# AIRI-Institute/HairFastGAN

Measured on AMD Instinct MI355X. Metric: stylegan2_generator_fwd_1024_images_per_sec, higher is better.
Workload: dtype f32 tensors + f32 accumulate; conv products as 3 fp16 MFMAs on (hi,lo)-split operands (fp32-class); 1 GPU; StyleGAN2 1024^2 generator forward (range 0->8), random W+, fresh noise per layer, HIP modulated-conv + upfirdn2d kernels (BASELINE.json configs[1]); batch_per_gpu=8, global_batch=8, parallelism=replica x1, weights=synthetic closed-form (oracle/synth.py), conv_precision=f16x3

## Files before the change

hairfastgan_amd/_lib.py:

```python
import ctypes
import os

_HERE = os.path.dirname(os.path.abspath(__file__))
LIB_PATH = os.environ.get("HAIRFAST_HIP_LIB") or os.path.join(_HERE, "csrc", "libhairfast_hip.so")

_f = ctypes.c_void_p
_i = ctypes.c_int
_ll = ctypes.c_longlong
_fl = ctypes.c_float
_st = ctypes.c_void_p

SIGNATURES = {
    "hf_upfirdn2d_f32": [_f, _f, _f, _i, _i, _i, _i, _i, _i, _i, _i, _i, _i, _i, _i, _i, _st],
    "hf_fused_bias_act_f32": [_f, _f, _f, _ll, _i, _i, _fl, _fl, _st],
    "hf_noise_bias_act_f32": [_f, _f, _f, _f, _f, _i, _i, _i, _ll, _fl, _fl, _st],
    "hf_modconv_prepare_f32": [_f, _f, _f, _i, _i, _i, _st],
    "hf_modulation_f32": [_f, _f, _ll, _f, _f, _i, _i, _i, _st],
    "hf_style_batch_f32": [_f, _f, _ll, _ll, _f, _i, _i, _i, _i, _i, _st],
    "hf_demod_f32": [_f, _f, _f, _i, _i, _i, _st],
    "hf_style_normalize_f32": [_f, _f, _i, _i, _i, _st],
    "hf_modconv3x3_f32": [_f, _f, _f, _f, _f, _f, _f, _ll, _f, _i, _i, _i, _i, _i, _fl, _fl, _f, _ll, _st],
    "hf_conv_split_weights_f16": [_f, _f, _f, _i, _i, _st],
    "hf_conv_split_weights_f16_taps": [_f, _f, _f, _i, _i, _i, _st],
    "hf_modconv3x3_small_f16_f32": [_f, _f, _f, _f, _i, _f, _f, _f, _f, _ll, _f, _i, _i, _i, _i, _i, _fl, _fl, _i, _i, _f, _ll, _st],
    "hf_modconv3x3_small_up_blur_f16_f32": [_f, _f, _f, _f, _f, _f, _i, _f, _f, _f, _f, _f, _ll, _f, _f, _i, _i, _i, _i, _i, _fl, _fl, _f, _ll, _st],
    "hf_conv1x1_f16_f32": [_f, _f, _f, _f, _f, _f, _i, _f, _f, _f, _f, _i, _f, _fl, _f, _i, _i, _i, _i, _i, _i, _i, _ll, _f, _ll, _st],
    "hf_modconv3x3_f16_f32": [_f, _f, _f, _f, _i, _f, _f, _f, _f, _ll, _f, _i, _i, _i, _i, _i, _fl, _fl, _st],
    "hf_modconv3x3_f16_rgb_f32": [_f, _f, _f, _f, _i, _f, _f, _f, _f, _ll, _f, _i, _i, _i, _i, _i, _fl, _fl, _f, _f, _f, _st],
    "hf_modconv3x3_f16_pre_image_f32": [_f, _f, _f, _f, _f, _i, _f, _f, _f, _ll, _f, _i, _i, _i, _i, _i, _fl, _fl, _f, _f, _f, _f, _f, _st],
    "hf_modconv3x3_f16_pre_f32": [_f, _f, _f, _f, _f, _i, _f, _f, _f, _ll, _f, _i, _i, _i, _i, _i, _fl, _fl, _f, _f, _f, _f, _f, _f, _st],
    "hf_modconv3x3_up_f16_pre_f32": [_f, _f, _f, _f, _f, _i, _f, _i, _i, _i, _i, _i, _i, _st],
    "hf_modconv3x3_up_f16_f32": [_f, _f, _f, _f, _i, _f, _f, _i, _i, _i, _i, _i, _i, _st],
    "hf_modconv3x3_up_blur_f16_f32": [_f, _f, _f, _f, _f, _f, _f, _f, _f, _f, ctypes.POINTER(ctypes.c_float),
                                      ctypes.POINTER(ctypes.c_float), _f, _f, _ll, _f, _f, _i, _i, _i, _i, _i, _fl, _fl, _st],
    "hf_modconv3x3_up_f32": [_f, _f, _f, _f, _f, _i, _i, _i, _i, _i, _i, _f, _ll, _st],
    "hf_modconv_up_pitch": [_i],
    "hf_blur_noise_bias_act_f32": [_f, _f, _f, _f, _f, _ll, _f, _i, _i, _i, _i, _i, _fl, _fl, _st],
    "hf_blur_noise_bias_act_split_f16": [_f, _f, _f, _f, _f, _f, _ll, _f, _f, _i, _i, _i, _i, _i, _fl, _fl, _st],
    "hf_torgb_f32": [_f, _f, _f, _f, _f, _f, _f, _i, _i, _i, _i, _st],
    "hf_conv_prepare_f32": [_f, _f, _i, _i, _i, _fl, _st],
    "hf_bn_fold_f32": [_f, _f, _f, _f, _f, _f, _f, _fl, _i, _st],
    "hf_conv2d_f32": [_f, _f, _f, _f, _f, _f, _f, _i, _f, _fl, _f, _i, _i, _i, _i, _i, _i, _i, _i, _ll, _f, _ll, _st],
    "hf_conv2d_f16_f32": [_f, _f, _f, _f, _f, _f, _i, _f, _f, _f, _f, _i, _f, _fl, _f, _i, _i, _i, _i, _i, _i, _i, _ll, _f, _ll, _st],
    "hf_split_activation_f16": [_f, _f, _f, _f, _f, _ll, _i, _i, _i, _st],
    "hf_split_activation_mod_f16": [_f, _f, _f, _f, _ll, _i, _i, _i, _st],
    "hf_plane_mean_f32": [_f, _f, _i, _i, _st],
    "hf_se_gate_f32": [_f, _f, _f, _f, _i, _i, _i, _st],
    "hf_scale_shortcut_add_f32": [_f, _f, _f, _f, _i, _i, _i, _i, _i, _i, _i, _st],
    "hf_upsample_bilinear_add_f32": [_f, _f, _f, _i, _i, _i, _i, _i, _st],
    "hf_adaptive_avgpool_f32": [_f, _f, _i, _i, _i, _i, _i, _i, _i, _i, _st],
    "hf_downscale2x_f32": [_f, _f, _i, _i, _i, _st],
    "hf_linear_f32": [_f, _f, _ll, _f, _f, _i, _i, _i, _fl, _st],
    "hf_equal_linear_f32": [_f, _f, _ll, _f, _f, _i, _i, _i, _fl, _i, _fl, _fl, _st],
    "hf_pixel_norm_f32": [_f, _f, _i, _i, _st],
    "hf_bicubic_down_f32": [_f, _f, _f, _ll, _i, _i, _i, _st],
    "hf_dilate_erode_f32": [_f, _f, _f, _ll, _i, _i, _i, _st],
    "hf_quantize_u8_f32": [_f, _f, _ll, _st],
    "hf_poisson_setup_u8": [_f, _f, _f, _f, _f, _i, _i, _i, _i, _st],
    "hf_poisson_jacobi_f32": [_f, _f, _f, _f, _i, _i, _i, _i, _i, _i, _st],
    "hf_poisson_finish_u8": [_f, _f, _f, _f, _i, _i, _i, _i, _st],
    "hf_resize_lanczos_u8": [_f, _f, _f, _i, _i, _i, _i, _i, _f, _f, _i, _f, _f, _i, _st],
    "hf_quad_bilinear_u8": [_f, _f, ctypes.POINTER(ctypes.c_double), _i, _i, _i, _i, _i, _st],
    "hf_quad_lanczos4_u8": [_f, _f, ctypes.POINTER(ctypes.c_double), _i, _i, _i, _i, _f, _f, _i, _st],
    "hf_quad_lanczos4_ratio": [],
    "hf_align_pad_blur_f32": [_f, _f, _f, _f, _i, _f, _f, _i, _i, _i, _i, _i, _i, _i, _st],
    "hf_align_pad_finish_u8": [_f, _f, _f, _f, _f, _f, _i, _i, _i, _st],
    "hf_u8_to_unit_f32": [_f, _f, _ll, _st],
    "hf_image_to_bytes_f32": [_f, _f, _i, _i, _i, _fl, _fl, _i, _i, _st],
    "hf_labels_to_rgb_i64": [_f, _f, _ll, _f, _i, _i, _st],
    "hf_maxpool3x3s2_f32": [_f, _f, _ll, _i, _i, _st],
    "hf_gate_f32": [_f, _f, _f, _f, _f, _fl, _ll, _i, _st],
    "hf_upsample_nearest_f32": [_f, _f, _ll, _i, _i, _i, _i, _st],
    "hf_parsing_mask_i64": [_f, _f, _f, _i, _i, _i, _i, _i, _i, _i, _i, _st],
    "hf_layernorm_f32": [_f, _f, _f, _f, _i, _i, _fl, _i, _fl, _st],
    "hf_layernorm_grouped_f32": [_f, _f, _f, _f, _i, _i, _i, _fl, _i, _fl, _st],
    "hf_modulate_f32": [_f, _f, _f, _f, _ll, _i, _fl, _st],
    "hf_sample_layernorm_f32": [_f, _f, _f, _f, _i, _i, _i, _ll, _fl, _fl, _f, _ll, _st],
    "hf_pixel_norm_dim1_f32": [_f, _f, _i, _i, _i, _st],
    "hf_axpby_bcast_f32": [_f, _f, _fl, _f, _fl, _ll, _ll, _st],
    "hf_add_bcast_f32": [_f, _f, _f, _ll, _ll, _st],
    "hf_label_conv3x3_f32": [_f, _f, _f, _f, _i, _i, _i, _i, _i, _i, _i, _i, _f, _st],
    "hf_ace_modulate_f32": [_f, _f, _f, _f, _f, _f, _f, _f, _f, _i, _i, _i, _i, _fl, _i, _st],
    "hf_conv2d_f16_split_f32": [_f, _f, _f, _f, _f, _f, _f, _f, _f, _f, _i, _f, _f, _f, _f, _i, _f, _fl, _f, _i, _i, _i, _i, _i, _i, _st],
    "hf_stem7x7s2_f16_f32": [_f, _f, _f, _f, _f, _f, _f, _fl, _i, _i, _i, _i, _i, _st],
    "hf_ace_modulate_table_f32": [_f, _f, _f, _f, _f, _f, _f, _f, _f, _f, _f, _i, _i, _i, _i, _i, _i, _i, _fl, _i, _i, _st],
    "hf_region_mean_f32": [_f, _f, _f, _i, _i, _i, _i, _i, _ll, _ll, _i, _i, _st],
    "hf_tanh_f32": [_f, _f, _ll, _st],
    "hf_channel_layernorm_f32": [_f, _f, _f, _f, _i, _ll, _fl, _st],
    "hf_mha_small_f32": [_f, _f, _i, _i, _i, _i, _st],
    "hf_quick_gelu_f32": [_f, _f, _ll, _st],
    "hf_debug_set_dispatch": [_i, _i],
    "hf_debug_last_path": [],
    "hf_debug_set_persistent_blocks": [_i],
    "hf_debug_set_tuning": [_i],
    "hf_set_batch_invariant": [_i],
    "hf_set_splitk_counters": [_f, _i],
# ... 49 lines not shown
```

hairfastgan_amd/_marshal.py:

```python
import functools
import os

import torch
import torch.nn.functional as F

from ._lib import check
from ._runtime import CANON_BATCH, plan_batch

SQRT2 = 2 ** 0.5

PROFILE = None


KERNEL_NAMES = {
    211: "conv_mfma_pipe<2,2,2,4>", 212: "conv_mfma_pipe<2,2,1,4>", 213: "conv_mfma_pipe<1,2,1,4>",
    214: "conv_mfma_pipe<2,2,2,2>", 215: "conv_mfma_pipe<1,1,2,2>", 216: "conv_mfma_pipe<1,4,1,4>",
    231: "conv_mfma_dma<2,2,2,4>", 232: "conv_mfma_dma<2,2,1,4>", 233: "conv_mfma_dma<1,2,1,4>", 234: "conv_mfma_dma<2,2,2,2>",
    244: "conv_mfma_pipe<2,2,2,2,stride2>", 245: "conv_mfma_pipe<1,1,2,2,stride2>",
    221: "conv_mfma_pipe<1,2,2,2,up>", 222: "conv_mfma_pipe<1,2,1,4,up>", 223: "conv_mfma_pipe<1,1,2,2,up>",
    224: "conv_mfma_pipe<1,2,2,4,up>", 225: "conv_mfma_pipe<1,1,1,4,up>", 300: "conv_mfma<1,1,2,2> split-K",
    581: "conv_mfma_h<1,2,2,4,up,pre>", 583: "conv_mfma_h<1,2,1,8,up,pre>",
    571: "conv_mfma_h<1,2,2,4,pre>", 572: "conv_mfma_h<2,2,1,8,pre>", 575: "conv_mfma_h<1,2,1,8,tw128,pre>",
    579: "conv_rows_h<32->32,strip64,pre>",
    551: "conv_mfma_h<1,2,2,4>", 552: "conv_mfma_h<2,2,1,8>", 553: "conv_mfma_h<1,2,1,8>", 555: "conv_mfma_h<1,2,1,8,tw128>",
# ... 326 lines not shown
    return out, raw, split


def modconv3x3_f16_pre(lib, st, act, wt_hi, wt_lo, nterms, d, noise, noise_w, bias, alpha=0.2, scale=SQRT2, rgb=None,
                       want_out=True, split_for=None):
    out, raw, split = _modconv3x3_f16_pre(lib, st, act, wt_hi, wt_lo, nterms, d, noise, noise_w, bias, alpha, scale, rgb, want_out,
                                          split_for)
    res = (out,) + (() if rgb is None else (raw,)) + (() if split_for is None else (split,))
    return res[0] if len(res) == 1 else res


def split_weights_small(lib, st, wt):
    taps, cin, cout = wt.shape
    w1 = _c(wt).permute(1, 0, 2).reshape(1, cin, taps * cout).contiguous()
    return conv_split_weights_f16(lib, st, w1)


def modconv3x3_small_supported(cin, cout, h, w, batch, upsample=False):
    if cin % 32 or cout % 64 or h * w > 1024:
        return False
    n = plan_batch(batch) * h * w
    if upsample:
        return h * w <= 64 or (h * w <= 256 and n <= 1024)
    return 256 < n <= 2048 or (n == 256 and h * w <= 64) or (h * w == 64 and CANON_BATCH * 64 <= n <= 2048)


def conv3x3_small_supported(cin, cout, h, w, batch):
    return cin % 32 == 0 and cout % 64 == 0 and h * w <= 256 and plan_batch(batch) * h * w <= 4096 and cin * cout >= 512 * 512


def modconv3x3_small(lib, st, x, w9, nterms, s, d, noise, noise_w, bias, cout, alpha=0.2, scale=SQRT2, upsample=False):
    x = _c(x)
    b, cin, h, w = x.shape
    hi, lo = w9
    n = lib.hf_modconv3x3_small_workspace_floats(b, cin, cout, h, w)
    ws = x.new_empty((max(n, 1),))
    if upsample:
        pitch = lib.hf_modconv_up_pitch(w)
        out = x.new_empty((b, cout, 2 * h + 1, pitch))
        noise = bias = noise_w = None
        nbs = 0
    else:
        pitch = 0
        out = x.new_empty((b, cout, h, w))
        noise, nbs = _noise_args(noise, b, h * w)
    code = _launch_profiled(
        lib, 2.0 * cin * cout * 9 * h * w * b,
        lambda: lib.hf_modconv3x3_small_f16_f32(_p(out), _p(x), _p(hi), _p(lo), nterms, _p(_c(s)), _p(_c(d)), _p(noise),
                                                _p(_c(noise_w)), nbs, _p(_c(bias)), b, cin, cout, h, w, alpha, scale,
                                                1 if upsample else 0, pitch, _p(ws), n, st),
        label="gemm_h tap-GEMM (small planes)")
    check(lib, code, "hf_modconv3x3_small_f16_f32")
    return out


SMALL_UP_FUSED = os.environ.get("HAIRFAST_SMALL_UP_FUSED", "1") != "0"


def small_up_blur_supported(h, w):
    return (8 * (2 * h + 3) * (2 * w + 3) + 72 * h * w) * 4 <= 150 * 1024


def modconv3x3_small_up_blur(lib, st, x, w9, nterms, s, d, blur_kernel, noise, noise_w, bias, cout, alpha=0.2, scale=SQRT2,
                             split_for=None):
    x = _c(x)
    b, cin, h, w = x.shape
    hi, lo = w9
    n = lib.hf_modconv3x3_small_workspace_floats(b, cin, cout, h, w)
    ws = x.new_empty((max(n, 1),))
    noise, nbs = _noise_args(noise, b, 4 * h * w)
    out = split = s_next = None
    if split_for is not None:
        s_next = _c(split_for[1])
        split = SplitActivation.empty(b, cout, 2 * h, 2 * w, x.device, want_lo=split_for[2] if len(split_for) > 2 else True,
                                      key=split_for[0])
    else:
        out = x.new_empty((b, cout, 2 * h, 2 * w))
    code = _launch_profiled(
        lib, 2.0 * cin * cout * 9 * h * w * b,
        lambda: lib.hf_modconv3x3_small_up_blur_f16_f32(_p(out), *_hl(split), _p(x), _p(hi), _p(lo), nterms, _p(_c(s)), _p(_c(d)),
                                                        _p(_c(blur_kernel)), _p(noise), _p(_c(noise_w)), nbs, _p(_c(bias)),
                                                        _p(s_next), b, cin, cout, h, w, alpha, scale, _p(ws), n, st),
        label="gemm_h tap-GEMM (small planes)")
    check(lib, code, "hf_modconv3x3_small_up_blur_f16_f32")
    return out if split_for is None else split


def modconv3x3_up_f16_supported(cin, cout, h, w, batch=None):
    if batch is not None and plan_batch(batch) * h * w < 512:
        return False
    return cin % 16 == 0 and cout % 32 == 0 and h * w >= (256 if cout % 64 == 0 else 512) and min(h, w) >= 2


def modconv3x3_up(lib, st, x, wt, s, d, blur_kernel, noise, noise_w, bias, alpha=0.2, scale=SQRT2, f16=None,
                  split_for=None, small=None):
    pre = isinstance(x, SplitActivation)
    if not pre:
        x = _c(x)
    b, cin, h, w = x.shape
    cout = wt.shape[2]
    pitch = lib.hf_modconv_up_pitch(w)
    if pre or small is None:
        tmp = torch.empty((b, cout, 2 * h + 1, pitch), dtype=torch.float32, device=(x.hi if pre else x).device)
    if pre:
        hi, lo, nterms = f16
        code = _launch_profiled(
# ... 811 lines not shown
```

hairfastgan_amd/csrc/api.hip:

```cpp
#include "hf_common.h"

extern "C" const char *hf_strerror(int code) {
  switch (code) {
    case HF_OK: return "ok";
    case HF_E_INVALID: return "invalid argument";
    case HF_E_LAUNCH: return "kernel launch failed";
    case HF_E_WORKSPACE: return "workspace too small";
    default: return "unknown error";
  }
}

extern "C" int hf_abi_version(void) { return 13; }

__global__ void hf_profile_marker_kernel() {}

extern "C" int hf_profile_marker(int id, void *stream) {
  if (id < 0 || id > 1023) return HF_E_INVALID;
  hipLaunchKernelGGL(hf_profile_marker_kernel, dim3(id + 1), dim3(64), 0, static_cast<hipStream_t>(stream));
  return hipGetLastError() == hipSuccess ? HF_OK : HF_E_LAUNCH;
}

extern "C" unsigned long long hf_f16_overflow_count_convh(int reset);
extern "C" unsigned long long hf_f16_overflow_count_blur(int reset);
extern "C" unsigned long long hf_f16_overflow_count_enc(int reset);
extern "C" unsigned long long hf_f16_overflow_count_gemm(int reset);
extern "C" unsigned long long hf_f16_overflow_count_stem(int reset);

extern "C" long long hf_f16_overflow_count(int reset) {
  return (long long)(hf_f16_overflow_count_convh(reset) + hf_f16_overflow_count_blur(reset) + hf_f16_overflow_count_enc(reset) +
                     hf_f16_overflow_count_gemm(reset) + hf_f16_overflow_count_stem(reset));
}
```

hairfastgan_amd/stylegan2/model.py:

```python
import math
import os
import random

import torch
from torch import nn
from torch.nn import functional as F

from .. import _marshal as M
from .._runtime import conv_nterms, conv_precision, lib, reference_rng_walk, require_gpu, run_guarded, stream
from .op import FusedLeakyReLU, fused_leaky_relu, upfirdn2d


FUSE_BLUR_MIN_H = int(os.environ.get("HAIRFAST_FUSE_BLUR_MIN_H", "128"))


class PixelNorm(nn.Module):
    def forward(self, input):
        require_gpu(input)
        return M.pixel_norm(lib(), stream(), input)


def make_kernel(k):
    k = torch.tensor(k, dtype=torch.float32)
    if k.ndim == 1:
# ... 72 lines not shown
        self.upsample = upsample
        self.downsample = downsample
        if upsample:
            factor = 2
            p = (len(blur_kernel) - factor) - (kernel_size - 1)
            self.blur = Blur(blur_kernel, pad=((p + 1) // 2 + factor - 1, p // 2 + 1), upsample_factor=factor)
        self.scale = 1 / math.sqrt(in_channel * kernel_size ** 2)
        self.padding = kernel_size // 2
        self.weight = nn.Parameter(torch.randn(1, out_channel, in_channel, kernel_size, kernel_size))
        self.modulation = EqualLinear(style_dim, in_channel, bias_init=1)
        self.demodulate = demodulate
        self._prep = None
        self._prep_f16 = None
        self._coeffs = None
        self.register_load_state_dict_post_hook(lambda m, _ik: m.invalidate())

    def invalidate(self):
        self._prep = self._prep_f16 = self._coeffs = None

    def __repr__(self):
        return (f"{self.__class__.__name__}({self.in_channel}, {self.out_channel}, {self.kernel_size}, "
                f"upsample={self.upsample}, downsample={self.downsample})")

    def prepared(self):
        w = self.weight
        key = (w.data_ptr(), None if w.is_inference() else w._version, w.device)
        if self._prep is None or self._prep[0] != key:
            require_gpu(w)
            wt, wsq = M.prepare_weights(lib(), stream(), w.detach())
            self._prep = (key, wt, wsq)
        return self._prep[1], self._prep[2]

    def prepared_f16(self):
        wt, _ = self.prepared()
        key = self._prep[0]
        if self._prep_f16 is None or self._prep_f16[0] != key:
            hi, lo = M.split_weights_f16(lib(), stream(), wt)
            self._prep_f16 = (key, hi, lo)
        return self._prep_f16[1], self._prep_f16[2]

    def prepared_small(self):
        wt, _ = self.prepared()
        key = self._prep[0]
        cached = self.__dict__.get("_prep_small")
        if cached is None or cached[0] != key:
            cached = self.__dict__["_prep_small"] = (key, M.split_weights_small(lib(), stream(), wt))
        return cached[1]

    def route_same_res(self, shape, plain=True):
        b, cin, h, w = shape
        cout = self.out_channel
        if conv_precision() == "f32":
            return "f32", False
        if plain and M.modconv3x3_small_supported(cin, cout, h, w, b):
            return "small", False
        if M.modconv3x3_f16_supported(cin, cout, h, w, batch=b):
            return "f16", not self.upsample and self.kernel_size == 3 and M.torgb_fusable(cin, cout, h, w)
        return "f32", False

    def route_up(self, shape, is_split=False, tail=True):
        b, cin, h, w = shape
        cout = self.out_channel
        if conv_precision() == "f32":
            return "f32"
        if h >= FUSE_BLUR_MIN_H and tail and M.modconv3x3_up_fused_supported(cin, cout, h, w) and self.blur_factors() is not None:
            return "fused"
        if not is_split and M.modconv3x3_small_supported(cin, cout, h, w, b, upsample=True):
            return "small"
        return "f16" if M.modconv3x3_up_f16_supported(cin, cout, h, w, batch=b) else "f32"

    def conv_same_res(self, input, wt, s, d, noise, noise_w, bias, alpha=0.2, scale=math.sqrt(2), rgb=None):
        kernel, _ = self.route_same_res(input.shape, plain=rgb is None)
        if kernel == "small":
            return M.modconv3x3_small(lib(), stream(), input, self.prepared_small(), conv_nterms(), s, d, noise, noise_w, bias,
                                      self.out_channel, alpha, scale)
        if kernel == "f16":
            hi, lo = self.prepared_f16()
            return M.modconv3x3_f16(lib(), stream(), input, hi, lo, conv_nterms(), s, d, noise, noise_w, bias, alpha, scale, rgb=rgb)
        assert rgb is None
        return M.modconv3x3(lib(), stream(), input, wt, s, d, noise, noise_w, bias, alpha, scale)

    def fuses_torgb(self, input):
        return self.route_same_res(input.shape, plain=False)[1]

    def blur_factors(self):
        k = self.blur.kernel
        key = (k.data_ptr(), k._version if not k.is_inference() else None)
        cached = self.__dict__.get("_blur_fac")
        if cached is None or cached[0] != key:
            if torch.cuda.is_current_stream_capturing():
                return None if cached is None else cached[1]
            cached = self.__dict__["_blur_fac"] = (key, M.blur_factors(k))
        return cached[1]

    def conv_up(self, input, wt, s, d, noise, noise_w, bias, alpha=0.2, scale=math.sqrt(2), split_for=None):
        route = self.route_up(input.shape, isinstance(input, M.SplitActivation),
                              tail=noise is not None and bias is not None and 0.0 <= alpha <= 1.0)
        if route == "fused":
            hi, lo = self.prepared_f16()
            return M.modconv3x3_up_fused(lib(), stream(), input, hi, lo, s, d, self.blur_factors(), noise, noise_w, bias, alpha, scale,
                                         split_for=None if split_for is None else split_for[1], nterms=conv_nterms())
        f16 = small = None
        if route == "small":
            small = (self.prepared_small(), conv_nterms())
        elif route == "f16":
            f16 = (*self.prepared_f16(), conv_nterms())
        return M.modconv3x3_up(lib(), stream(), input, wt, s, d, self.blur.kernel, noise, noise_w, bias, alpha, scale,
                               f16=f16, split_for=split_for, small=small)

    def style_coefficients(self, style):
        pre = self._coeffs
        if pre is not None and pre[0] == (style.data_ptr(), tuple(style.shape), tuple(style.stride())):
            return pre[1]
        wt, wsq = self.prepared()
        s = M.modulation(lib(), stream(), style, self.modulation.weight.detach(), self.modulation.bias.detach())
        d = None
        if self.demodulate:
            d = M.demod(lib(), stream(), s, wsq)
            M.style_normalize(lib(), stream(), s, d)
        return wt, s, d

    def forward(self, input, style):
        require_gpu(input, style)
        wt, s, d = self.style_coefficients(style)
        if self.kernel_size == 1:
            return M.torgb(lib(), stream(), input, wt, s, None, None, None)
        if self.upsample:
            if tuple(self.blur.pad) != (1, 1) or tuple(self.blur.kernel.shape) != (4, 4):
                raise NotImplementedError("fused upsampling path expects the [1,3,3,1] blur with pad (1,1)")
            return self.conv_up(input, wt, s, d, None, None, None)
        return self.conv_same_res(input, wt, s, d, None, None, None)


# ... 28 lines not shown
        self.noise = NoiseInjection()
        self.activate = FusedLeakyReLU(out_channel)

    def forward(self, input, style, noise=None):
        return self._run(input, style, noise, None)

    def forward_rgb(self, input, style, noise, rgb):
        return self._run(input, style, noise, rgb)

    def _run(self, input, style, noise, rgb):
        require_gpu(input, style, noise)
        conv = self.conv
        wt, s, d = conv.style_coefficients(style)
        b, _, h, w = input.shape
        oh, ow = (2 * h, 2 * w) if conv.upsample else (h, w)
        if noise is None:
            noise = input.new_empty(b, 1, oh, ow).normal_()
        act = self.activate
        if conv.upsample:
            assert rgb is None
            return conv.conv_up(input, wt, s, d, noise, self.noise.weight.detach(), act.bias.detach(),
                                act.negative_slope, act.scale)
        if rgb is None:
            return conv.conv_same_res(input, wt, s, d, noise, self.noise.weight.detach(), act.bias.detach(),
                                      act.negative_slope, act.scale)
        rgb_wt, rgb_s = rgb
        return conv.conv_same_res(input, wt, s, d, noise, self.noise.weight.detach(), act.bias.detach(),
                                  act.negative_slope, act.scale, rgb=(rgb_wt, rgb_s))

    def forward_split(self, input, style, noise, s_next, coeffs=None):
        pre = isinstance(input, M.SplitActivation)
        require_gpu(None if pre else input, style, noise)
        conv = self.conv
        assert conv.upsample
        wt, s, d = conv.style_coefficients(style) if coeffs is None else coeffs
        b, _, h, w = input.shape
        if noise is None:
            noise = style.new_empty(b, 1, 2 * h, 2 * w).normal_()
        act = self.activate
        return conv.conv_up(input, wt, s, d, noise, self.noise.weight.detach(), act.bias.detach(),
                            act.negative_slope, act.scale, split_for=(None, s_next, conv_precision() == "f16x3"))

    def forward_image(self, split, coeffs, noise, rgb, to_rgb, skip):
        conv, act = self.conv, self.activate
        _, s, d = coeffs
        b, _, h, w = split.shape
        if noise is None:
            noise = split.hi.new_empty(b, 1, h, w, dtype=torch.float32).normal_()
        require_gpu(noise, skip)
        hi, lo = conv.prepared_f16()
        return M.modconv3x3_f16_pre_image(lib(), stream(), split, hi, lo, conv_nterms(), d, noise, self.noise.weight.detach(),
                                          act.bias.detach(), rgb, to_rgb.bias.detach(), skip, to_rgb._skip_kernel(skip),
                                          act.negative_slope, act.scale)

    def forward_from_split(self, split, coeffs, noise=None, rgb=None, want_out=True, split_for=None):
        conv = self.conv
        assert not conv.upsample
        _, s, d = coeffs
        b, _, h, w = split.shape
        if noise is None:
            noise = split.hi.new_empty(b, 1, h, w, dtype=torch.float32).normal_()
        require_gpu(noise)
        act = self.activate
        hi, lo = conv.prepared_f16()
        return M._modconv3x3_f16_pre(lib(), stream(), split, hi, lo, conv_nterms(), d, noise, self.noise.weight.detach(),
                                     act.bias.detach(), act.negative_slope, act.scale, rgb=rgb, want_out=want_out,
                                     split_for=split_for)


def _observed(*modules):
    for m in modules:
        for sub in m.modules():
            if sub._forward_hooks or sub._forward_pre_hooks:
                return True
    return False


class ToRGB(nn.Module):
    def __init__(self, in_channel, style_dim, upsample=True, blur_kernel=[1, 3, 3, 1]):
        super().__init__()
        if upsample:
            self.upsample = Upsample(blur_kernel)
        self.conv = ModulatedConv2d(in_channel, 3, 1, style_dim, demodulate=False)
        self.bias = nn.Parameter(torch.zeros(1, 3, 1, 1))

    def _skip_kernel(self, skip):
        if skip is None:
            return None
        kern = self.upsample.kernel
        if tuple(kern.shape) != (4, 4) or self.upsample.factor != 2 or tuple(self.upsample.pad) != (2, 1):
            raise NotImplementedError("fused skip path expects the [1,3,3,1] x2 upsampler")
        return kern

    def forward(self, input, style, skip=None):
        require_gpu(input, style, skip)
        wt, s, _ = self.conv.style_coefficients(style)
        return M.torgb(lib(), stream(), input, wt, s, self.bias.detach(), skip, self._skip_kernel(skip))

    def coefficients(self, style):
        wt, s, _ = self.conv.style_coefficients(style)
        return wt, s

    def finish(self, raw, skip=None):
        require_gpu(raw, skip)
        slabs = raw.shape[1] // 3
        eye = getattr(self, "_eye", None)
# ... 130 lines not shown
        res = M.style_batch(lib(), stream(), lat, table, layout, total, mci, mco)
        for conv, row, (sv, dv) in zip(convs, rows, res):
            view = latent[:, row]
            conv._coeffs = ((view.data_ptr(), tuple(view.shape), tuple(view.stride())), (conv.prepared()[0], sv, dv))
        return convs

    def _fast_block(self, block, src, mid_shape, fuses, latent, noise, skip, up_coeffs, end_layer):
        conv_up, conv_same, to_rgb = self.convs[2 * block - 2], self.convs[2 * block - 1], self.to_rgbs[block - 1]
        i = 2 * block - 1
        coeffs = conv_same.conv.style_coefficients(latent[:, i + 1])
        split = conv_up.forward_split(src, latent[:, i], noise[2 * block - 1], coeffs[1],
                                      coeffs=up_coeffs if isinstance(src, M.SplitActivation) else None)
        rgb = to_rgb.coefficients(latent[:, i + 2]) if fuses else None
        is_last = block == self.log_size - 2
        s_up = None
        if not is_last and block + 1 <= end_layer:
            nup, nsame = self.convs[2 * block], self.convs[2 * block + 1]
            up_shape = (mid_shape[0], conv_same.conv.out_channel) + mid_shape[2:]
            next_mid = (mid_shape[0], nup.conv.out_channel, 2 * mid_shape[2], 2 * mid_shape[3])
            if (nup.conv.route_up(up_shape, is_split=True) != "f32" and nsame.conv.route_same_res(next_mid, plain=False)[0] == "f16"
                    and not _observed(nup, nsame)):
                up_coeffs = nup.conv.style_coefficients(latent[:, i + 2])
                s_up = up_coeffs[1]
        fused_rgb = rgb is not None and not _observed(to_rgb)
        want_out = not fused_rgb or (not is_last and s_up is None)
        if (fused_rgb and not want_out and s_up is None and skip is not None and M.image_fusable(mid_shape[1], conv_same.conv.out_channel, *mid_shape[2:])
                and conv_same.activate.bias is not None):
            image = conv_same.forward_image(split, coeffs, noise[2 * block], rgb, to_rgb, skip)
            if image is not None:
                return None, image, None, up_coeffs
        out, raw, split_in = conv_same.forward_from_split(split, coeffs, noise[2 * block], rgb=rgb if fused_rgb else None,
                                                          want_out=want_out, split_for=s_up)
        skip = to_rgb.finish(raw, skip) if raw is not None else to_rgb(out, latent[:, i + 2], skip)
        return out, skip, split_in, up_coeffs

    def _run_layers(self, latent, noise, layer_in, skip, start_layer, end_layer, return_latents):
        out = self.input(latent)
        if start_layer == 0:
            out = self.conv1(out, latent[:, 0], noise=noise[0])
            skip = self.to_rgb1(out, latent[:, 1])
        if end_layer == 0:
            return out, skip
        split_in = up_coeffs = None
        for block in range(1, self.log_size - 1):
            if block < start_layer:
                continue
            if block != start_layer and block > end_layer:
                return out, skip
            conv_up, conv_same, to_rgb = self.convs[2 * block - 2], self.convs[2 * block - 1], self.to_rgbs[block - 1]
            i = 2 * block - 1
            src = layer_in if block == start_layer else (split_in if split_in is not None else out)
            mid_shape = (src.shape[0], conv_up.conv.out_channel, 2 * src.shape[2], 2 * src.shape[3])
            kernel, fuses = conv_same.conv.route_same_res(mid_shape, plain=False)
            if kernel == "f16" and not _observed(conv_up, conv_same):
                out, skip, split_in, up_coeffs = self._fast_block(block, src, mid_shape, fuses, latent, noise, skip, up_coeffs, end_layer)
            else:
                assert not isinstance(src, M.SplitActivation)
                split_in = None
                out = conv_up(src, latent[:, i], noise=noise[2 * block - 1])
                if fuses and not _observed(conv_same, to_rgb):
                    out, raw = conv_same.forward_rgb(out, latent[:, i + 1], noise[2 * block], to_rgb.coefficients(latent[:, i + 2]))
                    skip = to_rgb.finish(raw, skip)
                else:
                    out = conv_same(out, latent[:, i + 1], noise=noise[2 * block])
                    skip = to_rgb(out, latent[:, i + 2], skip)
        image = skip
        return (image, latent) if return_latents else (image, None)
```

include/hairfast_hip.h:

```cpp
#ifndef HAIRFAST_HIP_H
#define HAIRFAST_HIP_H

#ifdef __cplusplus
extern "C" {
#endif

#define HF_OK 0
#define HF_E_INVALID (-1)
#define HF_E_LAUNCH (-2)
#define HF_E_WORKSPACE (-3)

#define HF_ACT_RESIDUAL_FIRST 16

const char *hf_strerror(int code);
int hf_abi_version(void);

int hf_upfirdn2d_f32(float *out, const float *in, const float *kernel, int major, int in_h, int in_w,
                     int kh, int kw, int up_x, int up_y, int down_x, int down_y, int pad_x0, int pad_x1,
                     int pad_y0, int pad_y1, void *stream);

int hf_fused_bias_act_f32(float *out, const float *x, const float *bias, long long n, int n_bias,
                          int step_b, float alpha, float scale, void *stream);

int hf_noise_bias_act_f32(float *out, const float *x, const float *noise, const float *noise_w,
// ... 79 lines not shown
                                     const float *noise, const float *noise_w, long long noise_bstride,
                                     const float *bias, const float *s_next, int batch, int channels, int in_h,
                                     int in_w, int in_pitch, float alpha, float scale, void *stream);

int hf_torgb_f32(float *out, const float *x, const float *wt, const float *s, const float *bias,
                 const float *skip, const float *kernel4x4, int batch, int cin, int h, int w,
                 void *stream);


int hf_conv_prepare_f32(float *wt, const float *weight, int cout, int cin, int k, float scale, void *stream);

int hf_bn_fold_f32(float *scale, float *shift, const float *gamma, const float *beta, const float *mean,
                   const float *var, const float *conv_bias, float eps, int n, void *stream);

int hf_conv2d_f32(float *out, const float *x, const float *wt, const float *in_scale, const float *in_shift,
                  const float *out_scale, const float *bias, int act, const float *slope, float alpha,
                  const float *residual, int batch, int cin, int cout, int h, int w, int k, int stride,
                  int groups, long long x_group_stride, float *workspace, long long workspace_floats,
                  void *stream);
long long hf_conv2d_workspace_floats(int batch, int cin, int cout, int h, int w, int k, int stride, int groups);

int hf_conv2d_f16_f32(float *out, const float *x, const void *x_hi, const void *x_lo, const void *wt_hi,
                      const void *wt_lo, int nterms, const float *in_scale, const float *in_shift,
                      const float *out_scale, const float *bias, int act, const float *slope, float alpha,
                      const float *residual, int batch, int cin, int cout, int h, int w, int stride, int groups,
                      long long x_group_stride, float *workspace, long long workspace_floats, void *stream);
long long hf_conv2d_f16_workspace_floats(int batch, int cin, int cout, int h, int w, int stride, int groups);
int hf_conv2d_f16_split_f32(float *out, void *out_hi, void *out_lo, const float *next_scale, const float *next_shift,
                            const float *x, const void *x_hi, const void *x_lo, const void *wt_hi, const void *wt_lo,
                            int nterms, const float *in_scale, const float *in_shift, const float *out_scale,
                            const float *bias, int act, const float *slope, float alpha, const float *residual, int batch,
                            int cin, int cout, int h, int w, int stride, void *stream);
int hf_scale_shortcut_add_split_f16(float *out, void *out_hi, void *out_lo, const float *next_scale, const float *next_shift,
                                    const float *r, const float *gate, const float *shortcut, int sc_stride, int batch, int channels,
                                    int oh, int ow, int sh, int sw, void *stream);
int hf_conv2d_f16_split_output_ok(int batch, int cin, int cout, int h, int w, int stride, int nterms, int presplit_input);
int hf_conv1x1_f16_f32(float *out, const float *x, const void *x_hi, const void *x_lo, const void *wt_hi,
                       const void *wt_lo, int nterms, const float *in_scale, const float *in_shift, const float *out_scale, const float *bias, int act,
                       const float *slope, float alpha, const float *residual, int batch, int cin, int cout, int h, int w,
                       int stride, int groups, long long x_group_stride, float *workspace, long long workspace_floats,
                       void *stream);
long long hf_conv1x1_f16_workspace_floats(int batch, int cin, int cout, int h, int w, int stride, int groups);
int hf_modconv3x3_small_f16_f32(float *out, const float *x, const void *w9_hi, const void *w9_lo, int nterms, const float *s,
                                const float *d, const float *noise, const float *noise_w, long long noise_bstride,
                                const float *bias, int batch, int cin, int cout, int h, int w, float alpha, float scale,
                                int upsample, int tmp_pitch, float *workspace, long long workspace_floats, void *stream);
long long hf_modconv3x3_small_workspace_floats(int batch, int cin, int cout, int h, int w);
int hf_modconv3x3_small_up_blur_f16_f32(float *out, void *out_hi, void *out_lo, const float *x, const void *w9_hi,
                                        const void *w9_lo, int nterms, const float *s, const float *d,
                                        const float *blur_kernel4x4, const float *noise, const float *noise_w,
                                        long long noise_bstride, const float *bias, const float *s_next, int batch, int cin,
                                        int cout, int h, int w, float alpha, float scale, float *workspace,
                                        long long workspace_floats, void *stream);
int hf_split_activation_f16(void *out_hi, void *out_lo, const float *x, const float *in_scale, const float *in_shift,
                            long long images, int channels, int h, int w, void *stream);

int hf_split_activation_mod_f16(void *out_hi, void *out_lo, const float *x, const float *scale, long long images,
                                int channels, int h, int w, void *stream);

int hf_plane_mean_f32(float *out, const float *x, int planes, int hw, void *stream);
int hf_se_gate_f32(float *gate, const float *pooled, const float *fc1, const float *fc2, int batch, int channels,
                   int reduced, void *stream);
int hf_scale_shortcut_add_f32(float *out, const float *r, const float *gate, const float *shortcut,
                              int sc_stride, int batch, int channels, int oh, int ow, int sh, int sw,
                              void *stream);
int hf_upsample_bilinear_add_f32(float *out, const float *x, const float *y, int planes, int h, int w, int oh,
                                 int ow, void *stream);
int hf_adaptive_avgpool_f32(float *out, const float *x, int batch, int channels, int h, int w, int oh, int ow,
                            int out_channels_total, int out_channel_offset, void *stream);
int hf_downscale2x_f32(float *out, const float *x, int planes, int h, int w, void *stream);
int hf_linear_f32(float *out, const float *x, long long x_stride, const float *w, const float *bias, int batch,
                  int in_features, int out_features, float scale, void *stream);
int hf_equal_linear_f32(float *out, const float *x, long long x_stride, const float *w, const float *bias, int batch,
                        int in_features, int out_features, float lr_mul, int fused_lrelu, float alpha, float act_scale,
                        void *stream);
int hf_pixel_norm_f32(float *out, const float *x, int rows, int dim, void *stream);
int hf_maxpool3x3s2_f32(float *out, const float *x, long long planes, int h, int w, void *stream);
int hf_gate_f32(float *out, const float *x, const float *logit, const float *add_plane, const float *add_bcast,
                float plus_one, long long planes, int hw, void *stream);
int hf_upsample_nearest_f32(float *out, const float *x, long long planes, int h, int w, int oh, int ow, void *stream);
int hf_parsing_mask_i64(long long *out, const float *logits, const int *remap, int images, int classes, int h, int w,
                        int full_h, int full_w, int out_h, int out_w, void *stream);

int hf_sample_layernorm_f32(float *out, const float *x, const float *gamma, const float *beta, int batch, int channels,
                            int hw, long long x_batch_stride, float eps, float slope, float *workspace,
                            long long workspace_floats, void *stream);
long long hf_sample_layernorm_workspace_floats(int batch, int channels, int hw);
int hf_bicubic_down_f32(float *out, const float *x, const float *k1d, long long planes, int h, int w, int factor,
                        void *stream);
int hf_dilate_erode_f32(float *dilated, float *eroded, const float *mask, long long planes, int h, int w, int radius,
                        void *stream);

int hf_quantize_u8_f32(unsigned char *out, const float *x, long long n, void *stream);
int hf_poisson_setup_u8(float *b, float *x0, const unsigned char *src, const unsigned char *tgt, const unsigned char *mask,
                        int images, int channels, int h, int w, void *stream);
int hf_poisson_jacobi_f32(float *x_out, const float *x_in, const float *b, const unsigned char *mask, int images, int channels,
                          int h, int w, int sweeps, int tblock, void *stream);
int hf_poisson_finish_u8(unsigned char *out, const float *x, const unsigned char *tgt, const unsigned char *mask, int images,
                         int channels, int h, int w, void *stream);

int hf_resize_lanczos_u8(unsigned char *out, unsigned char *mid, const unsigned char *in, int planes, int h_in, int w_in,
                         int h_out, int w_out, const int *bounds_x, const int *kk_x, int ksize_x, const int *bounds_y,
                         const int *kk_y, int ksize_y, void *stream);
int hf_quad_bilinear_u8(unsigned char *out, const unsigned char *src, const double *coef8, int planes, int h, int w, int oh,
                        int ow, void *stream);
int hf_quad_lanczos4_u8(unsigned char *out, const unsigned char *src, const double *coef8, int planes, int h, int w, int osize,
// ... 61 lines not shown
```

Measured before the change: 1807 images/s.

## Add direct MFMA 3x3 modconv kernel for small planes with split-cin reduction

Adds a new kernel for 4x4, 8x8 and 16x16 same-resolution modulated convs. It stages pre-split f16 activations into LDS per wave and runs the 3x3 taps directly as 32x32x16 MFMAs. Input channels are split across 8 waves and reduced through LDS, with noise, bias, lrelu and optional next-layer split fused into the epilogue. The early-resolution path is routed through it in place of the tap-GEMM small kernel. The cost is an extra split-activation launch per layer and a new code path with fallbacks.

```diff
diff --git a/hairfastgan_amd/_lib.py b/hairfastgan_amd/_lib.py
--- a/hairfastgan_amd/_lib.py
+++ b/hairfastgan_amd/_lib.py
@@ -42,6 +42,8 @@
     "hf_bn_fold_f32": [_f, _f, _f, _f, _f, _f, _f, _fl, _i, _st],
     "hf_conv2d_f32": [_f, _f, _f, _f, _f, _f, _f, _i, _f, _fl, _f, _i, _i, _i, _i, _i, _i, _i, _i, _ll, _f, _ll, _st],
     "hf_conv2d_f16_f32": [_f, _f, _f, _f, _f, _f, _i, _f, _f, _f, _f, _i, _f, _fl, _f, _i, _i, _i, _i, _i, _i, _i, _ll, _f, _ll, _st],
+    "hf_modconv3x3_small_direct_supported": [_i, _i, _i, _i, _i],
+    "hf_modconv3x3_small_direct_f16_f32": [_f, _f, _f, _f, _f, _f, _f, _i, _f, _f, _f, _ll, _f, _f, _i, _i, _i, _i, _i, _fl, _fl, _i, _st],
     "hf_split_activation_f16": [_f, _f, _f, _f, _f, _ll, _i, _i, _i, _st],
     "hf_split_activation_mod_f16": [_f, _f, _f, _f, _ll, _i, _i, _i, _st],
     "hf_plane_mean_f32": [_f, _f, _i, _i, _st],
diff --git a/hairfastgan_amd/_marshal.py b/hairfastgan_amd/_marshal.py
--- a/hairfastgan_amd/_marshal.py
+++ b/hairfastgan_amd/_marshal.py
@@ -402,6 +402,50 @@
         label="gemm_h tap-GEMM (small planes)")
     check(lib, code, "hf_modconv3x3_small_f16_f32")
     return out
+
+
+DIRECT_PLANES = (4, 8, 16)
+
+
+def modconv3x3_small_direct_supported(lib, cin, cout, h, w, batch):
+    return (h == w and w in DIRECT_PLANES and plan_batch(batch) * h * w <= 2048
+            and bool(lib.hf_modconv3x3_small_direct_supported(batch, cin, cout, h, w)))
+
+
+def modconv3x3_small_direct(lib, st, act, wt_hi, wt_lo, nterms, d, noise, noise_w, bias, alpha=0.2, scale=SQRT2, want_out=True,
+                            split_for=None, tiles=0):
+    b, cin, h, w = act.shape
+    cout = wt_hi.shape[3]
+    dev = act.hi.device
+    noise, nbs = _noise_args(noise, b, h * w)
+    if not want_out and split_for is None:
+        raise ValueError("want_out=False needs split_for=")
+    out = torch.empty((b, cout, h, w), dtype=torch.float32, device=dev) if want_out else None
+    split = s_next = None
+    if split_for is not None:
+        s_next = _c(split_for)
+        split = SplitActivation.empty(b, cout, h, w, dev, want_lo=nterms == 3)
+    nparts = 2 if nterms == 3 else 1
+    nb = (float(b) * h * w * (2.0 * nparts * cin + (4.0 * cout if want_out else 0.0) + (2.0 * nparts * cout if split is not None else 0.0))
+          + 2.0 * nparts * 9 * cin * cout)
+    code = _launch_profiled(
+        lib, 2.0 * cin * cout * 9 * h * w * b,
+        lambda: lib.hf_modconv3x3_small_direct_f16_f32(_p(out), *_hl(split), _p(act.hi), _p(act.lo), _p(wt_hi), _p(wt_lo), nterms,
+                                                       _p(_c(d)), _p(noise), _p(_c(noise_w)), nbs, _p(_c(bias)), _p(s_next), b, cin,
+                                                       cout, h, w, alpha, scale, tiles, st),
+        label="conv_small_h (small planes, direct)", nbytes=nb)
+    if code == -1:
+        return None
+    check(lib, code, "hf_modconv3x3_small_direct_f16_f32")
+    return out, split
+
+
+def split_activation_mod(lib, st, x, s, want_lo=True):
+    x = _c(x)
+    b, c, h, w = x.shape
+    split = SplitActivation.empty(b, c, h, w, x.device, want_lo=want_lo)
+    check(lib, lib.hf_split_activation_mod_f16(*_hl(split), _p(x), _p(_c(s)), b, c, h, w, st), "hf_split_activation_mod_f16")
+    return split
 
 
 SMALL_UP_FUSED = os.environ.get("HAIRFAST_SMALL_UP_FUSED", "1") != "0"
diff --git a/hairfastgan_amd/csrc/api.hip b/hairfastgan_amd/csrc/api.hip
--- a/hairfastgan_amd/csrc/api.hip
+++ b/hairfastgan_amd/csrc/api.hip
@@ -1,3 +1,6 @@
+#ifndef __HIPCC__
+#include "convsmall.hip"
+#endif
 #include "hf_common.h"
 
 extern "C" const char *hf_strerror(int code) {
@@ -25,8 +28,9 @@
 extern "C" unsigned long long hf_f16_overflow_count_enc(int reset);
 extern "C" unsigned long long hf_f16_overflow_count_gemm(int reset);
 extern "C" unsigned long long hf_f16_overflow_count_stem(int reset);
+extern "C" unsigned long long hf_f16_overflow_count_convsmall(int reset);
 
 extern "C" long long hf_f16_overflow_count(int reset) {
   return (long long)(hf_f16_overflow_count_convh(reset) + hf_f16_overflow_count_blur(reset) + hf_f16_overflow_count_enc(reset) +
-                     hf_f16_overflow_count_gemm(reset) + hf_f16_overflow_count_stem(reset));
+                     hf_f16_overflow_count_gemm(reset) + hf_f16_overflow_count_stem(reset) + hf_f16_overflow_count_convsmall(reset));
 }
diff --git a/hairfastgan_amd/csrc/convsmall.hip b/hairfastgan_amd/csrc/convsmall.hip
--- /dev/null
+++ b/hairfastgan_amd/csrc/convsmall.hip
@@ -0,0 +1,327 @@
+#define HF_WANT_F16_SPLIT
+#include "conv_common.h"
+
+using namespace hf_detail;
+
+namespace {
+
+typedef _Float16 half8 __attribute__((ext_vector_type(8)));
+constexpr int NWAVES = 8;
+
+__device__ __forceinline__ void wait_vmem() {
+#if defined(__HIPCC__)
+  asm volatile("s_waitcnt vmcnt(0)" ::: "memory");
+#endif
+}
+__device__ __forceinline__ void wait_lds() {
+#if defined(__HIPCC__)
+  asm volatile("s_waitcnt lgkmcnt(0)" ::: "memory");
+#endif
+}
+
+struct SmallParams {
+  float *out;
+  void *oh, *ol;
+  const void *xh, *xl;
+  const float *d, *noise, *noise_w, *bias, *s_next;
+  long long noise_bstride;
+  int batch, cin, cout;
+  int std_tail;
+  float alpha, scale;
+};
+
+template <int NTERMS, int PG, int LGW>
+struct SmallShape {
+  static constexpr int W = 1 << LGW, PLANE = W * W;
+  static constexpr int IMS = PLANE < 32 ? 32 / PLANE : 1;
+  static constexpr int IMG_TILES = PLANE < 32 ? 1 : PLANE / 32;
+  static_assert(PG >= 1 && PG <= IMG_TILES && IMG_TILES % PG == 0, "a block takes whole rows of one image");
+  static constexpr int R = PLANE < 32 ? W : PG * 32 / W;
+  static constexpr int PITCH = W + 1;
+  static constexpr int IMU = (R + 2) * PITCH + 1;
+  static constexpr int SU = IMS * IMU;
+  static constexpr int NPART = NTERMS == 3 ? 2 : 1;
+  static constexpr int WAVE_UNITS = NPART * 2 * SU;
+  static constexpr int NE = (2 * SU + 63) / 64;
+  static constexpr int TR = PG >= 2 ? 2 : 1;
+  static constexpr size_t stage_bytes = (size_t)NWAVES * WAVE_UNITS * 16;
+  static constexpr size_t reduce_bytes = (size_t)TR * NWAVES * 16 * 64 * sizeof(float);
+  static constexpr size_t lds_bytes = stage_bytes > reduce_bytes ? stage_bytes : reduce_bytes;
+};
+
+template <int NTERMS, int PG, int LGW>
+__global__ __launch_bounds__(64 * NWAVES, 2) void conv_small_h(const SmallParams P, const _Float16 *__restrict__ wth,
+                                                               const _Float16 *__restrict__ wtl) {
+#pragma clang fp contract(on)
+  using S = SmallShape<NTERMS, PG, LGW>;
+  constexpr int W = S::W, PLANE = S::PLANE, IMS = S::IMS, R = S::R, PITCH = S::PITCH, IMU = S::IMU, SU = S::SU;
+  constexpr int NPART = S::NPART, NE = S::NE, TR = S::TR;
+
+  HF_DYN_LDS;
+  half8 *lds = reinterpret_cast<half8 *>(hf_dyn_lds);
+  const int tid = threadIdx.x, lane = tid & 63, wave = tid >> 6;
+  const int li = lane & 31, lh = lane >> 5;
+  const int co0 = (int)blockIdx.x * 32;
+  const int grp = (int)blockIdx.y;
+  const int b0 = PLANE < 32 ? grp * IMS : grp / (S::IMG_TILES / PG);
+  const int tg = PLANE < 32 ? 0 : grp % (S::IMG_TILES / PG);
+  const int y0 = tg * R;
+
+  const int nchunks = P.cin >> 4;
+  const int cbase = nchunks / NWAVES, crem = nchunks % NWAVES;
+  const int c_begin = wave * cbase + min(wave, crem), c_end = c_begin + cbase + (wave < crem ? 1 : 0);
+
+  half8 *stage = lds + wave * S::WAVE_UNITS;
+  const unsigned stage_addr = hf_lds_addr(stage);
+  int e_src[NE];
+#pragma unroll
+  for (int e = 0; e < NE; ++e) {
+    const int i = lane + e * 64;
+    const int kg = i / SU, u = i - kg * SU;
+    const int im = u / IMU, r = u - im * IMU;
+    const int rr = r / PITCH, cc = r - rr * PITCH;
+    const int y = y0 - 1 + rr, x = cc - 1, b = b0 + im;
+    e_src[e] = -2;
+    if (i < 2 * SU) {
+      const bool inside = cc > 0 && rr < R + 2 && y >= 0 && y < W && b < P.batch;
+      e_src[e] = inside ? (((b * (P.cin >> 3) + kg) * PLANE + y * W + x) * 16) : -1;
+    }
+  }
+  {
+    half8 z;
+#pragma unroll
+    for (int k = 0; k < 8; ++k) z[k] = (_Float16)0.0f;
+#pragma unroll
+    for (int e = 0; e < NE; ++e)
+      if (e_src[e] == -1) {
+#pragma unroll
+        for (int part = 0; part < NPART; ++part) stage[part * 2 * SU + lane + e * 64] = z;
+      }
+  }
+  auto dma_x = [&](int chunk) {
+    const unsigned cofs = (unsigned)chunk * 2u * PLANE * 16u;
+#pragma unroll
+    for (int e = 0; e < NE; ++e) {
+      const bool inside = e_src[e] >= 0;
+      const unsigned off = inside ? (unsigned)e_src[e] + cofs : 0u;
+      hf_glds16_raw_s_if(inside, P.xh, off, stage_addr + (unsigned)(e * 64) * 16u);
+      if (NTERMS == 3) hf_glds16_raw_s_if(inside, P.xl, off, stage_addr + (unsigned)(2 * SU + e * 64) * 16u);
+    }
+  };
+
+  int pbase[PG];
+#pragma unroll
+  for (int t = 0; t < PG; ++t) {
+    const int p = PLANE < 32 ? (li & (PLANE - 1)) : ((tg * PG + t) * 32 + li);
+    const int im = PLANE < 32 ? li / PLANE : 0;
+    pbase[t] = lh * SU + im * IMU + ((p >> LGW) - y0) * PITCH + (p & (W - 1));
+  }
+
+  f32x16 vsum[PG];
+#pragma unroll
+  for (int t = 0; t < PG; ++t)
+#pragma unroll
+    for (int r = 0; r < 16; ++r) vsum[t][r] = 0.0f;
+
+  const half8 *wh8 = reinterpret_cast<const half8 *>(wth) + (long long)lh * P.cout + co0 + li;
+  const half8 *wl8 = NTERMS == 3 ? reinterpret_cast<const half8 *>(wtl) + (long long)lh * P.cout + co0 + li : nullptr;
+  const long long tap_units = 2LL * P.cout;
+
+  for (int c = c_begin; c < c_end; ++c) {
+    wait_lds();
+    dma_x(c);
+    f32x16 acc[PG];
+#pragma unroll
+    for (int t = 0; t < PG; ++t)
+#pragma unroll
+      for (int r = 0; r < 16; ++r) acc[t][r] = 0.0f;
+    half8 ah[3][3], al[3][3];
+    auto load_row = [&](int ky) {
+#pragma unroll
+      for (int kx = 0; kx < 3; ++kx) {
+        const long long u = ((long long)c * 9 + ky * 3 + kx) * tap_units;
+        ah[ky][kx] = wh8[u];
+        if (NTERMS == 3) al[ky][kx] = wl8[u];
+      }
+    };
+    load_row(0);
+    load_row(1);
+    wait_vmem();
+#pragma unroll
+    for (int ky = 0; ky < 3; ++ky) {
+      if (ky == 0) load_row(2);
+#pragma unroll
+      for (int kx = 0; kx < 3; ++kx) {
+#pragma unroll
+        for (int t = 0; t < PG; ++t) {
+          const int u = pbase[t] + ky * PITCH + kx;
+          const half8 bh = stage[u];
+          acc[t] = __builtin_amdgcn_mfma_f32_32x32x16_f16(ah[ky][kx], bh, acc[t], 0, 0, 0);
+          if (NTERMS == 3) {
+            const half8 bl = stage[2 * SU + u];
+            acc[t] = __builtin_amdgcn_mfma_f32_32x32x16_f16(ah[ky][kx], bl, acc[t], 0, 0, 0);
+            acc[t] = __builtin_amdgcn_mfma_f32_32x32x16_f16(al[ky][kx], bh, acc[t], 0, 0, 0);
+          }
+        }
+      }
+    }
+#pragma unroll
+    for (int t = 0; t < PG; ++t) vsum[t] += acc[t];
+  }
+
+  const float w_unscale = *reinterpret_cast<const float *>(wth + 9LL * P.cin * P.cout);
+  const float nw = P.noise ? P.noise_w[0] : 0.0f;
+  float *red = reinterpret_cast<float *>(hf_dyn_lds);
+  bool ovf_any = false;
+#pragma unroll
+  for (int t0 = 0; t0 < PG; t0 += TR) {
+    __syncthreads();
+#pragma unroll
+    for (int tl = 0; tl < TR; ++tl)
+#pragma unroll
+      for (int r = 0; r < 16; ++r) red[((tl * NWAVES + wave) * 16 + r) * 64 + lane] = vsum[t0 + tl][r];
+    __syncthreads();
+    const int tl = TR == 2 ? wave >> 2 : 0, q = wave & 3;
+    if (TR == 1 && wave >= 4) continue;
+    float sum[4];
+#pragma unroll
+    for (int k = 0; k < 4; ++k) {
+      float v = red[((tl * NWAVES + 0) * 16 + 4 * q + k) * 64 + lane];
+#pragma unroll
+      for (int v8 = 1; v8 < NWAVES; ++v8) v += red[((tl * NWAVES + v8) * 16 + 4 * q + k) * 64 + lane];
+      sum[k] = v;
+    }
+    const int t = t0 + tl;
+    const int p = PLANE < 32 ? (li & (PLANE - 1)) : ((tg * PG + t) * 32 + li);
+    const int b = b0 + (PLANE < 32 ? li / PLANE : 0);
+    const bool valid = b < P.batch;
+    const int bc = valid ? b : b0;
+    const int c4 = co0 + 8 * q + 4 * lh;
+    const float nz = P.noise ? P.noise[(long long)bc * P.noise_bstride + p] : 0.0f;
+    float v[4];
+    if (P.std_tail) {
+      const float nws = nw * P.scale;
+      float nzv = nws * nz;
+      HF_OPAQUE_F32(nzv);
+#pragma unroll
+      for (int k = 0; k < 4; ++k) {
+        const float dm = (P.d ? P.d[(long long)bc * P.cout + c4 + k] : 1.0f) * w_unscale * P.scale;
+        const float bs = P.bias[c4 + k] * P.scale;
+        const float o = fmaf(sum[k], dm, nzv + bs);
+        v[k] = fmaxf(o, o * P.alpha);
+      }
+    } else {
+      const float nzv = nw * nz;
+#pragma unroll
+      for (int k = 0; k < 4; ++k) {
+        const float dm = (P.d ? P.d[(long long)bc * P.cout + c4 + k] : 1.0f) * w_unscale;
+        float o = sum[k] * dm;
+        o = o + nzv + (P.bias ? P.bias[c4 + k] : 0.0f);
+        v[k] = P.bias ? hf_lrelu(o, P.alpha, P.scale) : o;
+      }
+    }
+    if (P.out && valid) {
+#pragma unroll
+      for (int k = 0; k < 4; ++k) P.out[((long long)b * P.cout + c4 + k) * PLANE + p] = v[k];
+    }
+    if (P.oh) {
+      hf_half4 h4, l4;
+      bool ovf = false;
+#pragma unroll
+      for (int k = 0; k < 4; ++k) {
+        const float vs = v[k] * (P.s_next ? P.s_next[(long long)bc * P.cout + c4 + k] : 1.0f);
+        _Float16 hv, lv;
+        hf_split_f16(vs, hv, lv, ovf);
+        h4[k] = hv;
+        l4[k] = lv;
+      }
+      if (valid) {
+        ovf_any = ovf_any || ovf;
+        const long long off = (((long long)b * (P.cout >> 3) + (c4 >> 3)) * PLANE + p) * 16 + (c4 & 4) * 2;
+        *reinterpret_cast<hf_half4 *>(static_cast<char *>(P.oh) + off) = h4;
+        if (P.ol) *reinterpret_cast<hf_half4 *>(static_cast<char *>(P.ol) + off) = l4;
+      }
+    }
+  }
+  if (P.oh) hf_note_overflow(ovf_any);
+}
+
+int pick_tiles(int img_tiles, int co_tiles, int batch, int forced) {
+  if (forced) return forced;
+  int pg = img_tiles > 4 ? 4 : img_tiles;
+  while (pg > 1 && (long long)co_tiles * batch * (img_tiles / pg) < 192) pg >>= 1;
+  return pg;
+}
+
+template <int NTERMS, int PG, int LGW>
+bool small_resources_ok() {
+#if defined(__HIPCC__)
+  static const bool ok = [] {
+    hipFuncAttributes a{};
+    if (hipFuncGetAttributes(&a, reinterpret_cast<const void *>(&conv_small_h<NTERMS, PG, LGW>)) != hipSuccess) {
+      (void)hipGetLastError();
+      return false;
+    }
+    return a.localSizeBytes == 0 && a.numRegs <= 256;
+  }();
+  return ok;
+#else
+  return true;
+#endif
+}
+
+template <int NTERMS, int PG, int LGW>
+int launch_small(const SmallParams &P, const _Float16 *wth, const _Float16 *wtl, hipStream_t st) {
+  using S = SmallShape<NTERMS, PG, LGW>;
+  static_assert(S::lds_bytes <= 160 * 1024, "one block per CU at most: 160 KiB of LDS");
+  if (!small_resources_ok<NTERMS, PG, LGW>()) return HF_E_INVALID;
+  const int groups = S::PLANE < 32 ? hf_cdiv(P.batch, S::IMS) : P.batch * (S::IMG_TILES / PG);
+  const dim3 grid(P.cout / 32, groups);
+  if (grid.y > 65535) return HF_E_INVALID;
+  hipLaunchKernelGGL((conv_small_h<NTERMS, PG, LGW>), grid, dim3(64 * NWAVES), S::lds_bytes, st, P, wth, wtl);
+  return hf_launch_status();
+}
+
+template <int NTERMS>
+int launch_small_form(int lgw, int pg, const SmallParams &P, const _Float16 *wth, const _Float16 *wtl, hipStream_t st) {
+  if (lgw == 2 && pg == 1) return launch_small<NTERMS, 1, 2>(P, wth, wtl, st);
+  if (lgw == 3 && pg == 1) return launch_small<NTERMS, 1, 3>(P, wth, wtl, st);
+  if (lgw == 3 && pg == 2) return launch_small<NTERMS, 2, 3>(P, wth, wtl, st);
+  if (lgw == 4 && pg == 1) return launch_small<NTERMS, 1, 4>(P, wth, wtl, st);
+  if (lgw == 4 && pg == 2) return launch_small<NTERMS, 2, 4>(P, wth, wtl, st);
+  if (lgw == 4 && pg == 4) return launch_small<NTERMS, 4, 4>(P, wth, wtl, st);
+  return HF_E_INVALID;
+}
+
+}
+
+extern "C" int hf_modconv3x3_small_direct_supported(int batch, int cin, int cout, int h, int w) {
+  return !(g_h_tune & 64) && batch > 0 && cin > 0 && cout > 0 && h == w && (w == 4 || w == 8 || w == 16) && (cin % 16) == 0 &&
+         (cout % 32) == 0 && (long long)batch * cin * h * w * 2 < (1LL << 31) && (long long)batch * 8 <= 65535;
+}
+
+extern "C" int hf_modconv3x3_small_direct_f16_f32(float *out, void *out_hi, void *out_lo, const void *x_hi, const void *x_lo,
+                                                  const void *wt_hi, const void *wt_lo, int nterms, const float *d,
+                                                  const float *noise, const float *noise_w, long long noise_bstride,
+                                                  const float *bias, const float *s_next, int batch, int cin, int cout, int h,
+                                                  int w, float alpha, float scale, int tiles, void *stream) {
+  if ((!out && !out_hi) || !x_hi || !wt_hi || batch <= 0 || cin <= 0 || cout <= 0 || (nterms != 1 && nterms != 3) ||
+      (nterms == 3 && (!x_lo || !wt_lo || (out_hi && !out_lo))) || (noise && !noise_w))
+    return HF_E_INVALID;
+  if (!hf_modconv3x3_small_direct_supported(batch, cin, cout, h, w) || tiles < 0)
+    return HF_E_INVALID;
+  const int lgw = ilog2(w), img_tiles = h * w < 32 ? 1 : h * w / 32;
+  if (tiles && (tiles > img_tiles || tiles > 4 || (tiles & (tiles - 1)))) return HF_E_INVALID;
+  SmallParams P{};
+  P.out = out; P.oh = out_hi; P.ol = nterms == 3 ? out_lo : nullptr; P.xh = x_hi; P.xl = nterms == 3 ? x_lo : nullptr;
+  P.d = d; P.noise = noise; P.noise_w = noise_w; P.bias = bias; P.s_next = s_next; P.noise_bstride = noise_bstride;
+  P.batch = batch; P.cin = cin; P.cout = cout; P.alpha = alpha; P.scale = scale;
+  P.std_tail = (bias && alpha >= 0.0f && alpha <= 1.0f && scale > 0.0f) ? 1 : 0;
+  const int pg = pick_tiles(img_tiles, cout / 32, batch, tiles);
+  const _Float16 *hi = static_cast<const _Float16 *>(wt_hi), *lo = static_cast<const _Float16 *>(wt_lo);
+  const int rc = with_nterms(nterms, [&](auto nt) { return launch_small_form<decltype(nt)::value>(lgw, pg, P, hi, lo, (hipStream_t)stream); });
+  if (rc == HF_OK) note_path(8, pg);
+  return rc;
+}
+
+extern "C" unsigned long long hf_f16_overflow_count_convsmall(int reset) { return hf_f16_overflow_read_tu(reset); }
diff --git a/hairfastgan_amd/stylegan2/model.py b/hairfastgan_amd/stylegan2/model.py
--- a/hairfastgan_amd/stylegan2/model.py
+++ b/hairfastgan_amd/stylegan2/model.py
@@ -148,6 +148,8 @@
         cout = self.out_channel
         if conv_precision() == "f32":
             return "f32", False
+        if M.modconv3x3_small_direct_supported(lib(), cin, cout, h, w, b):
+            return "direct", False
         if plain and M.modconv3x3_small_supported(cin, cout, h, w, b):
             return "small", False
         if M.modconv3x3_f16_supported(cin, cout, h, w, batch=b):
@@ -167,6 +169,14 @@
 
     def conv_same_res(self, input, wt, s, d, noise, noise_w, bias, alpha=0.2, scale=math.sqrt(2), rgb=None):
         kernel, _ = self.route_same_res(input.shape, plain=rgb is None)
+        if kernel == "direct":
+            assert rgb is None
+            split = M.split_activation_mod(lib(), stream(), input, s, want_lo=conv_nterms() == 3)
+            out = self.conv_direct(split, d, noise, noise_w, bias, alpha, scale)
+            if out is not None:
+                return out
+            b, cin, h, w = input.shape
+            kernel = "small" if M.modconv3x3_small_supported(cin, self.out_channel, h, w, b) else "f32"
         if kernel == "small":
             return M.modconv3x3_small(lib(), stream(), input, self.prepared_small(), conv_nterms(), s, d, noise, noise_w, bias,
                                       self.out_channel, alpha, scale)
@@ -175,6 +185,11 @@
             return M.modconv3x3_f16(lib(), stream(), input, hi, lo, conv_nterms(), s, d, noise, noise_w, bias, alpha, scale, rgb=rgb)
         assert rgb is None
         return M.modconv3x3(lib(), stream(), input, wt, s, d, noise, noise_w, bias, alpha, scale)
+
+    def conv_direct(self, split, d, noise, noise_w, bias, alpha=0.2, scale=math.sqrt(2)):
+        hi, lo = self.prepared_f16()
+        res = M.modconv3x3_small_direct(lib(), stream(), split, hi, lo, conv_nterms(), d, noise, noise_w, bias, alpha, scale)
+        return None if res is None else res[0]
 
     def fuses_torgb(self, input):
         return self.route_same_res(input.shape, plain=False)[1]
@@ -309,6 +324,16 @@
         return M.modconv3x3_f16_pre_image(lib(), stream(), split, hi, lo, conv_nterms(), d, noise, self.noise.weight.detach(),
                                           act.bias.detach(), rgb, to_rgb.bias.detach(), skip, to_rgb._skip_kernel(skip),
                                           act.negative_slope, act.scale)
+
+    def forward_direct(self, split, coeffs, noise=None):
+        conv, act = self.conv, self.activate
+        assert not conv.upsample
+        _, s, d = coeffs
+        b, _, h, w = split.shape
+        if noise is None:
+            noise = split.hi.new_empty(b, 1, h, w, dtype=torch.float32).normal_()
+        require_gpu(noise)
+        return conv.conv_direct(split, d, noise, self.noise.weight.detach(), act.bias.detach(), act.negative_slope, act.scale)
 
     def forward_from_split(self, split, coeffs, noise=None, rgb=None, want_out=True, split_for=None):
         conv = self.conv
@@ -545,9 +570,21 @@
             src = layer_in if block == start_layer else (split_in if split_in is not None else out)
             mid_shape = (src.shape[0], conv_up.conv.out_channel, 2 * src.shape[2], 2 * src.shape[3])
             kernel, fuses = conv_same.conv.route_same_res(mid_shape, plain=False)
+            done = False
             if kernel == "f16" and not _observed(conv_up, conv_same):
                 out, skip, split_in, up_coeffs = self._fast_block(block, src, mid_shape, fuses, latent, noise, skip, up_coeffs, end_layer)
-            else:
+                done = True
+            elif kernel == "direct" and not _observed(conv_up, conv_same):
+                assert not isinstance(src, M.SplitActivation)
+                split_in = None
+                coeffs = conv_same.conv.style_coefficients(latent[:, i + 1])
+                split = conv_up.forward_split(src, latent[:, i], noise[2 * block - 1], coeffs[1])
+                direct = conv_same.forward_direct(split, coeffs, noise[2 * block])
+                if direct is not None:
+                    out = direct
+                    skip = to_rgb(out, latent[:, i + 2], skip)
+                    done = True
+            if not done:
                 assert not isinstance(src, M.SplitActivation)
                 split_in = None
                 out = conv_up(src, latent[:, i], noise=noise[2 * block - 1])
diff --git a/include/hairfast_hip.h b/include/hairfast_hip.h
--- a/include/hairfast_hip.h
+++ b/include/hairfast_hip.h
@@ -155,6 +155,12 @@
                                         long long noise_bstride, const float *bias, const float *s_next, int batch, int cin,
                                         int cout, int h, int w, float alpha, float scale, float *workspace,
                                         long long workspace_floats, void *stream);
+int hf_modconv3x3_small_direct_supported(int batch, int cin, int cout, int h, int w);
+int hf_modconv3x3_small_direct_f16_f32(float *out, void *out_hi, void *out_lo, const void *x_hi, const void *x_lo,
+                                       const void *wt_hi, const void *wt_lo, int nterms, const float *d, const float *noise,
+                                       const float *noise_w, long long noise_bstride, const float *bias, const float *s_next,
+                                       int batch, int cin, int cout, int h, int w, float alpha, float scale, int tiles,
+                                       void *stream);
 int hf_split_activation_f16(void *out_hi, void *out_lo, const float *x, const float *in_scale, const float *in_shift,
                             long long images, int channels, int h, int w, void *stream);
 
```

Result: faster. 1832 images/s, median of 6 (+1.4%).
